# myungsub/meta-interpolation

Measured on AMD Instinct MI355X. Metric: inner-loop steps/sec, higher is better.
Workload: dtype f32 (3x3 convolutions: Winograd F(4x4) / F(2x2) on exact-f32 MFMAs, csrc/winograd4.h + winograd.hip; weight gradients and 5x5 / 7x7 / direct layers on csrc/convk*.hip: bf16x6 split operands, f32 accumulate; 51-tap op on 8-bit frames: exact integer frames x bf16x3 split taps, f32 accumulate); 1 GPU; c2_sepconv_256x448_b4_s5; plugin=sepconv, tasks_per_gpu=4, global_meta_batch=4, inner_steps=5, frame=256x448x3, inner_rule=lslr+SGD, seeded_weights=default, parallelism=task-parallel x1, 1 all-reduce of outer grads

## Files before the change

include/savfi_hip.h:

```cpp
#ifndef SAVFI_HIP_H_
#define SAVFI_HIP_H_

#include <stddef.h>
#include <stdint.h>

#ifdef __cplusplus
extern "C" {
#endif

#define SAVFI_ABI_VERSION 23

#define SAVFI_OK            0
#define SAVFI_E_NULL       (-1)
#define SAVFI_E_SHAPE      (-2)
#define SAVFI_E_UNSUPPORTED (-3)
#define SAVFI_E_TOOBIG     (-4)

int savfi_version(void);

int savfi_sepconv_fwd_f32(const float* in, const float* v, const float* h, float* out,
                          int B, int C, int Ho, int Wo, int K, void* stream);

int savfi_sepconv_bwd_f32(const float* in, const float* v, const float* h, const float* gO,
                          float* gI, float* gV, float* gH,
                          int B, int C, int Ho, int Wo, int K, void* stream);
// ... 104 lines not shown
                                    int Hs, int Ws, int oy0, int ox0, int Hw, int Ww, int align_corners, void* stream);
int savfi_upsample2x_window_bwd_masked_f32(const float* gout, const float* y, float slope, float* gin, int planes, int H, int W,
                                           int sy0, int sx0, int Hs, int Ws, int oy0, int ox0, int Hw, int Ww, int align_corners,
                                           void* stream);

int64_t savfi_conv3x3_workspace_floats(int N, int Ci, int Co, int H, int W, int pad, int mode);
int savfi_conv3x3_f32(const float* x, const float* w, const float* bias, float* out, float* workspace,
                      int N, int Ci, int Co, int H, int W, int pad, int mode, float slope, void* stream);

int64_t savfi_conv3x3_tasks_workspace_floats(int N, int T, int Ci, int Co, int H, int W, int pad, int mode);
int savfi_conv3x3_tasks_f32(const float* x, const float* w, const float* bias, float* out, float* workspace,
                            int N, int T, int Ci, int Co, int H, int W, int pad, int mode, float slope, void* stream);

int64_t savfi_conv3x3_filter_floats(int T, int Ci, int Co, int mode);
int64_t savfi_conv3x3_f4_workgroups(int N, int Ci, int Co, int H, int W, int pad, int mode);
int savfi_conv3x3_filters_form_f32(const float* w, float* u_fwd, float* u_bwd, int T, int Ci, int Co, int form, void* stream);
int savfi_conv3x3_filters_multi_form_f32(const float* const* w, float* const* u_fwd, float* const* u_bwd, const int* T, const int* Ci,
                                         const int* Co, const int* form, int n, void* stream);
int savfi_conv3x3_dgrad_masked_form_f32(const float* gy, const float* u, const float* mask, float mask_slope, float* gx, float* workspace,
                                        int N, int T, int Ci, int Co, int H, int W, int pad, int form, void* stream);
int savfi_conv3x3_filters_f32(const float* w, float* u_fwd, float* u_bwd, int T, int Ci, int Co, void* stream);
int savfi_conv3x3_filters_multi_f32(const float* const* w, float* const* u_fwd, float* const* u_bwd, const int* T, const int* Ci,
                                    const int* Co, int n, void* stream);
int64_t savfi_conv3x3_tasks_pre_workspace_floats(int N, int T, int Ci, int Co, int H, int W, int pad, int mode);
int savfi_conv3x3_tasks_pre_f32(const float* x, const float* u, const float* bias, float* out, float* workspace,
                                int N, int T, int Ci, int Co, int H, int W, int pad, int mode, float slope, void* stream);
int savfi_conv3x3_dgrad_masked_f32(const float* gy, const float* u, const float* mask, float mask_slope, float* gx,
                                   float* workspace, int N, int T, int Ci, int Co, int H, int W, int pad, void* stream);

int savfi_conv3x3_unit16_supported(int N, int T, int Ci, int Co, int H, int W, int pad);
// ... 5 lines not shown

int64_t savfi_conv3x3_wgrad_workspace_floats(int N, int Ci, int Co, int H, int W, int pad);
int savfi_conv3x3_wgrad_f32(const float* x, const float* gz, float* gw, float* workspace, int N, int Ci, int Co,
                            int H, int W, int pad, void* stream);

int64_t savfi_conv3x3_wgrad_tasks_workspace_floats(int N, int T, int Ci, int Co, int H, int W, int pad);
int savfi_conv3x3_wgrad_tasks_f32(const float* x, const float* gz, float* gw, float* workspace, int N, int T, int Ci,
                                  int Co, int H, int W, int pad, void* stream);

int64_t savfi_conv3x3_wgrad_wino_tasks_workspace_floats(int N, int T, int Ci, int Co, int H, int W, int pad);
int savfi_conv3x3_wgrad_wino_tasks_f32(const float* x, const float* gz, float* gw, float* workspace, int N, int T, int Ci,
                                       int Co, int H, int W, int pad, void* stream);
int64_t savfi_conv3x3_wgrad_wino_tasks_bias_workspace_floats(int N, int T, int Ci, int Co, int H, int W, int pad);
int savfi_conv3x3_wgrad_wino_tasks_bias_f32(const float* x, const float* gz, float* gw, float* gb, float* workspace, int N, int T, int Ci,
                                            int Co, int H, int W, int pad, void* stream);

int64_t savfi_convk_filter_floats(int T, int Ci, int Co, int K, int mode);
int savfi_convk_filters_f32(const float* w, float* p_fwd, float* p_bwd, int T, int Ci, int Co, int K, void* stream);
int savfi_convk_filters_multi_f32(const float* const* w, float* const* p_fwd, float* const* p_bwd, const int* T, const int* Ci,
                                  const int* Co, const int* K, int n, void* stream);
int savfi_convk_tasks_pre_f32(const float* x, const float* packed, const float* bias, float* out, int N, int T, int Ci,
                              int Co, int H, int W, int K, int pad, int mode, float slope, int precise, void* stream);
int savfi_convk_dgrad_masked_f32(const float* gy, const float* packed, const float* mask, float mask_slope, float* gx, int N, int T,
                                 int Ci, int Co, int H, int W, int K, int pad, int precise, void* stream);
int savfi_convk_tasks_pre_reflect_f32(const float* x, const float* packed, const float* bias, float* out, int N, int T, int Ci,
                                      int Co, int H, int W, int K, int pad, int mode, float slope, int precise, int reflect,
                                      void* stream);
int savfi_reflect_pad_bwd_f32(const float* gp, float* gx, int planes, int H, int W, int pad, void* stream);
int savfi_reflect_pad_bwd_add_f32(const float* gp, const float* add, float* gx, int planes, int H, int W, int pad, void* stream);
int savfi_reflect_pad_fwd_f32(const float* x, float* xp, int planes, int H, int W, int pad, void* stream);
// ... 37 lines not shown
```

meta-interpolation_amd/_hip.py:

```python
import ctypes
import os
import re
from ctypes import c_double, c_float, c_int, c_int64, c_void_p, POINTER

_PKG_DIR = os.path.dirname(os.path.abspath(__file__))
LIB_PATH = os.environ.get("SAVFI_HIP_LIB") or os.path.join(_PKG_DIR, "lib", "libsavfi_hip.so")
HEADER_PATH = os.path.join(os.path.dirname(_PKG_DIR), "include", "savfi_hip.h")

RULE_SGD, RULE_ADAM, RULE_ADAMAX_LSLR, RULE_ADAMAX_MSGD = 0, 1, 2, 3
LR_SCALAR, LR_ELEMENT = 0, 1
SSIM_RANGE_PER_ROW, SSIM_RANGE_BATCH, SSIM_RANGE_FIXED = 0, 1, 2
SEPCONV_PARTITION_WS, SEPCONV_PARTITION_X6, SEPCONV_PARTITION_FP32 = 0, 1, 2
ABI_VERSION = 23

_ERRORS = {-1: "SAVFI_E_NULL (a required pointer is NULL)",
           -2: "SAVFI_E_SHAPE (bad or inconsistent dimension)",
           -3: "SAVFI_E_UNSUPPORTED",
           -4: "SAVFI_E_TOOBIG (index arithmetic would overflow)"}


class SavfiHipError(RuntimeError):
    pass


_P = c_void_p
_PP = POINTER(c_void_p)
_I64P = POINTER(c_int64)
_FP = POINTER(c_float)
# ... 38 lines not shown
    "savfi_l1_mse_f32": [c_int, _P, _P, _P, _P, c_int, c_int64, _P],
    "savfi_l1_mse_bwd_f32": [c_int, _P, _P, _P, _P, c_int, c_int64, _P],
    "savfi_ssim_scratch_floats": [c_int, c_int, c_int, c_int],
    "savfi_ssim_loss_f32": [_P, _P, _P, _P, _P, c_int, c_int, c_int, c_int, c_int, _P],
    "savfi_ssim_loss_bwd_f32": [_P, _P, _P, _P, _P, c_int, c_int, c_int, c_int, _P],
    "savfi_psnr_ssim_scratch_bytes": [c_int, c_int, c_int, c_int],
    "savfi_psnr_ssim_f32": [_P, _P, _P, _P, _P, c_int, c_int, c_int, c_int, _P],
    "savfi_upsample2x_fwd_f32": [_P, _P, c_int, c_int, c_int, c_int, _P],
    "savfi_upsample2x_bwd_f32": [_P, _P, c_int, c_int, c_int, c_int, _P],
    "savfi_conv3x3_workspace_floats": [c_int] * 7,
    "savfi_conv3x3_f32": [_P, _P, _P, _P, _P, c_int, c_int, c_int, c_int, c_int, c_int, c_int, c_float, _P],
    "savfi_conv3x3_tasks_workspace_floats": [c_int] * 8,
    "savfi_conv3x3_tasks_f32": [_P, _P, _P, _P, _P, c_int, c_int, c_int, c_int, c_int, c_int, c_int, c_int, c_float, _P],
    "savfi_conv3x3_filter_floats": [c_int] * 4,
    "savfi_conv3x3_f4_workgroups": [c_int] * 7,
    "savfi_conv3x3_filters_form_f32": [_P, _P, _P, c_int, c_int, c_int, c_int, _P],
    "savfi_conv3x3_filters_multi_form_f32": [_P, _P, _P, _P, _P, _P, _P, c_int, _P],
    "savfi_conv3x3_dgrad_masked_form_f32": [_P, _P, _P, c_float, _P, _P, c_int, c_int, c_int, c_int, c_int, c_int, c_int, c_int, _P],
    "savfi_conv3x3_filters_f32": [_P, _P, _P, c_int, c_int, c_int, _P],
    "savfi_conv3x3_tasks_pre_workspace_floats": [c_int] * 8,
    "savfi_conv3x3_tasks_pre_f32": [_P, _P, _P, _P, _P, c_int, c_int, c_int, c_int, c_int, c_int, c_int, c_int, c_float, _P],
    "savfi_conv3x3_unit16_supported": [c_int] * 7,
    "savfi_conv3x3_in_unit16_supported": [c_int] * 7,
    "savfi_conv3x3_dgrad_in_unit16_f32": [_P, _P, _P, c_int, c_int, c_int, c_int, c_int, c_int, c_int, _P],
    "savfi_conv3x3_tasks_pre_unit16_f32": [_P, _P, _P, _P, c_int, c_int, c_int, c_int, c_int, c_int, c_int, c_float, _P],
    "savfi_conv3x3_wgrad_tasks_workspace_floats": [c_int] * 7,
    "savfi_conv3x3_wgrad_tasks_f32": [_P, _P, _P, _P, c_int, c_int, c_int, c_int, c_int, c_int, c_int, _P],
    "savfi_conv3x3_wgrad_wino_tasks_workspace_floats": [c_int] * 7,
    "savfi_conv3x3_wgrad_wino_tasks_f32": [_P, _P, _P, _P, c_int, c_int, c_int, c_int, c_int, c_int, c_int, _P],
    "savfi_conv3x3_wgrad_wino_tasks_bias_workspace_floats": [c_int] * 7,
    "savfi_conv3x3_wgrad_wino_tasks_bias_f32": [_P, _P, _P, _P, _P, c_int, c_int, c_int, c_int, c_int, c_int, c_int, _P],
    "savfi_conv3x3_wgrad_workspace_floats": [c_int] * 6,
    "savfi_conv3x3_wgrad_f32": [_P, _P, _P, _P, c_int, c_int, c_int, c_int, c_int, c_int, _P],
    "savfi_convk_filter_floats": [c_int] * 5,
    "savfi_convk_filters_f32": [_P, _P, _P, c_int, c_int, c_int, c_int, _P],
    "savfi_convk_filters_multi_f32": [_P, _P, _P, _P, _P, _P, _P, c_int, _P],
    "savfi_conv3x3_filters_multi_f32": [_P, _P, _P, _P, _P, _P, c_int, _P],
    "savfi_convk_tasks_pre_f32": [_P, _P, _P, _P] + [c_int] * 9 + [c_float, c_int, _P],
    "savfi_convk_tasks_pre_reflect_f32": [_P, _P, _P, _P] + [c_int] * 9 + [c_float, c_int, c_int, _P],
    "savfi_convk_wgrad_tasks_reflect_f32": [_P, _P, _P, _P] + [c_int] * 10 + [_P],
    "savfi_reflect_pad_bwd_f32": [_P, _P, c_int, c_int, c_int, c_int, _P],
    "savfi_reflect_pad_fwd_f32": [_P, _P, c_int, c_int, c_int, c_int, _P],
    "savfi_reflect_pad_bwd_add_f32": [_P, _P, _P, c_int, c_int, c_int, c_int, _P],
    "savfi_convk_wgrad_workspace_floats": [c_int] * 8,
    "savfi_convk_wgrad_sums_bias": [c_int] * 8,
    "savfi_convk_wgrad_tasks_bias_f32": [_P, _P, _P, _P, _P] + [c_int] * 9 + [_P],
# ... 166 lines not shown
```

meta-interpolation_amd/csrc/wgrad.hip:

```cpp
#include "common.h"

namespace {

typedef float f32x4 __attribute__((ext_vector_type(4)));

constexpr int GNT = 256;
constexpr int GCO = 32, GCI = 32, GSEG = 64;
constexpr int GP = 68;
constexpr int G_FLOATS = GCO * GP;
constexpr int X_FLOATS = 3 * GCI * GP;
constexpr int BUF_FLOATS = G_FLOATS + X_FLOATS;
constexpr int TILE_FLOATS = 2 * 2 * 9 * 256;
constexpr int LDS_FLOATS_G = (2 * BUF_FLOATS > TILE_FLOATS) ? 2 * BUF_FLOATS : TILE_FLOATS;

struct WgradArgs {
  const float* x;
  const float* gz;
  float* partial;
  int Ci, Co, H, W, Ho, Wo, pad, rows, nseg, nrowchunk, cibs;
  int T;
};

struct Staged {
  float g[8], x[3][8], halo;
// ... 273 lines not shown
constexpr int WW_BLOCK_FLOATS = WW_CB * WW_CB * 9;
#ifndef WW_DOUBLE
#define WW_DOUBLE 0
#endif
constexpr int WW_LDS_FLOATS = (WW_DOUBLE ? 2 : 1) * WW_BUF;

struct WWArgs {
  const float* x;
  const float* gz;
  float* partial;
  int Ci, Co, H, W, Ho, Wo, pad, T, cibs;
  int ty_cnt, tx_cnt, cpr;
  int chunks_total;
  int chunks_per_split;
  float* bias_partial;
};

}

__device__ f32x4 savfi_wg_buffer_load_x4(i32x4w rsrc, int voffset, int soffset, int aux) __asm("llvm.amdgcn.raw.buffer.load.v4f32");
__device__ f32x2w savfi_wg_buffer_load_x2(i32x4w rsrc, int voffset, int soffset, int aux) __asm("llvm.amdgcn.raw.buffer.load.v2f32");

namespace {

__device__ __forceinline__ i32x4w ww_rsrc(const float* base, unsigned bytes) {
  const unsigned long long p = reinterpret_cast<unsigned long long>(base);
  i32x4w r;
  r.x = (int)(unsigned)p; r.y = (int)(unsigned)(p >> 32); r.z = (int)bytes; r.w = 0x00020000;
  return r;
}
// ... 75 lines not shown
    t[12 + cc] = d[4 + cc] - d[12 + cc];
  }
#pragma unroll
  for (int r = 0; r < 4; ++r)
    *reinterpret_cast<f32x4*>(vbuf + (r * WW_CB + ch) * WW_PY + 4 * tl) =
        (f32x4){t[4 * r] - t[4 * r + 2], t[4 * r + 1] + t[4 * r + 2], t[4 * r + 2] - t[4 * r + 1], t[4 * r + 1] - t[4 * r + 3]};
  const float g00 = c.g[0], g01 = c.g[1], g10 = c.g[2], g11 = c.g[3];
  if (bias_acc) *bias_acc += (g00 + g01) + (g10 + g11);
  const float s0[2] = {g00, g01}, s1[2] = {g00 + g10, g01 + g11}, s2[2] = {g00 - g10, g01 - g11}, s3[2] = {g10, g11};
  *reinterpret_cast<f32x4*>(ybuf + (0 * WW_CB + ch) * WW_PY + 4 * tl) = (f32x4){s0[0], s0[0] + s0[1], s0[0] - s0[1], s0[1]};
  *reinterpret_cast<f32x4*>(ybuf + (1 * WW_CB + ch) * WW_PY + 4 * tl) = (f32x4){s1[0], s1[0] + s1[1], s1[0] - s1[1], s1[1]};
  *reinterpret_cast<f32x4*>(ybuf + (2 * WW_CB + ch) * WW_PY + 4 * tl) = (f32x4){s2[0], s2[0] + s2[1], s2[0] - s2[1], s2[1]};
  *reinterpret_cast<f32x4*>(ybuf + (3 * WW_CB + ch) * WW_PY + 4 * tl) = (f32x4){s3[0], s3[0] + s3[1], s3[0] - s3[1], s3[1]};
}

template <bool BIAS>
__global__ __launch_bounds__(256, WW_DOUBLE ? 2 : 4) void wino_wgrad3x3(WWArgs a) {
  extern __shared__ __attribute__((aligned(16))) float lds[];
  const int tid = threadIdx.x, lane = tid & 63, w = __builtin_amdgcn_readfirstlane(tid >> 6);
  const int tl = tid & 7, ch = tid >> 3;
  const int task = blockIdx.z;
  const int cob = blockIdx.y / a.cibs, cib = blockIdx.y - cob * a.cibs;
  const int q0 = blockIdx.x * a.chunks_per_split, q1 = min(q0 + a.chunks_per_split, a.chunks_total);
  const int ci = cib * WW_CB + ch, co = cob * WW_CB + ch;

  f32x4 acc[4][2][2];
#pragma unroll
  for (int c = 0; c < 4; ++c)
#pragma unroll
    for (int i = 0; i < 2; ++i)
#pragma unroll
// ... 46 lines not shown
        for (int i = 0; i < 2; ++i)
#pragma unroll
          for (int j = 0; j < 2; ++j) acc[c][i][j] = __builtin_amdgcn_mfma_f32_16x16x4f32(ya[i][c], va[j][c], acc[c][i][j], 0, 0, 0);
      __builtin_amdgcn_sched_barrier(0);
    }
  }
  __syncthreads();
  if (do_bias) {
    auto dpp = [](float v, auto ctrl) {
      return __builtin_bit_cast(float, __builtin_amdgcn_update_dpp(0, __builtin_bit_cast(int, v), decltype(ctrl)::value, 0xf, 0xf, true));
    };
    float bsum = *bias_slot();
    bsum += dpp(bsum, std::integral_constant<int, 0xB1>{});
    bsum += dpp(bsum, std::integral_constant<int, 0x4E>{});
    bsum += dpp(bsum, std::integral_constant<int, 0x141>{});
    if (tl == 0) a.bias_partial[(((size_t)task * gridDim.x + blockIdx.x) * (gridDim.y / a.cibs) + cob) * WW_CB + ch] = bsum;
  }

  const float sr = (w == 1 || w == 2) ? 0.5f : 1.f;
  float* ex = lds;
  float* out = a.partial + (((size_t)task * gridDim.x + blockIdx.x) * gridDim.y + blockIdx.y) * WW_BLOCK_FLOATS;
#pragma unroll
  for (int i = 0; i < 2; ++i) {
#pragma unroll
    for (int j = 0; j < 2; ++j) {
      f32x4 u0, u1, u2;
#pragma unroll
      for (int e = 0; e < 4; ++e) {
        const float m0 = acc[0][i][j][e], m1 = acc[1][i][j][e], m2 = acc[2][i][j][e], m3 = acc[3][i][j][e];
        const float h = 0.5f * (m1 + m2);
        u0[e] = sr * (m0 + h);
        u1[e] = sr * (0.5f * (m1 - m2));
        u2[e] = sr * (h - m3);
      }
      float* p = ex + ((w * 3) * 2 + j) * 256 + lane * 4;
      *reinterpret_cast<f32x4*>(p) = u0;
      *reinterpret_cast<f32x4*>(p + 2 * 256) = u1;
      *reinterpret_cast<f32x4*>(p + 4 * 256) = u2;
    }
    __syncthreads();
    for (int item = tid; item < 3 * 2 * 256; item += 256) {
      const int reg = item & 3, ln = (item >> 2) & 63, j = (item >> 8) & 1, b = item >> 9;
      const float* p = ex + (b * 2 + j) * 256 + ln * 4 + reg;
      const float u_0 = p[0], u_1 = p[3 * 2 * 256], u_2 = p[2 * 3 * 2 * 256], u_3 = p[3 * 3 * 2 * 256];
      const int cor = 16 * i + 4 * (ln >> 4) + reg, cic = 16 * j + (ln & 15);
      float* o = out + (cor * WW_CB + cic) * 9 + b;
      o[0] = u_0 + u_1 + u_2;
      o[3] = u_1 - u_2;
      o[6] = u_1 + u_2 - u_3;
    }
    __syncthreads();
  }
}

__global__ __launch_bounds__(256) void wino_wgrad_reduce2(const float* __restrict__ stage2, float* __restrict__ gw, int Co, int Ci,
                                                          int cibs, int ntiles, int ngroups) {
  const int e = blockIdx.x * 256 + threadIdx.x;
  if (e >= Co * Ci * 9) return;
  stage2 += (size_t)blockIdx.y * ngroups * ntiles * WW_BLOCK_FLOATS;
  gw += (size_t)blockIdx.y * Co * Ci * 9;
  const int k = e % 9, ci = (e / 9) % Ci, co = e / (9 * Ci);
// ... 56 lines not shown
  if (!ww_plan(p, N, T, Ci, Co, H, W, pad)) return SAVFI_E_SHAPE;
  return p.partial_floats + p.stage2_floats;
}

extern "C" int64_t savfi_conv3x3_wgrad_wino_tasks_bias_workspace_floats(int N, int T, int Ci, int Co, int H, int W, int pad) {
  const int64_t base = savfi_conv3x3_wgrad_wino_tasks_workspace_floats(N, T, Ci, Co, H, W, pad);
  if (base < 0) return base;
  WWPlan p;
  ww_plan(p, N, T, Ci, Co, H, W, pad);
  return base + (int64_t)T * p.nsplit * p.cobs * WW_CB;
}

static int wino_wgrad_tasks(const float* x, const float* gz, float* gw, float* gb, float* workspace, int N, int T, int Ci, int Co, int H,
                            int W, int pad, void* stream);

extern "C" int savfi_conv3x3_wgrad_wino_tasks_f32(const float* x, const float* gz, float* gw, float* workspace, int N, int T,
                                                  int Ci, int Co, int H, int W, int pad, void* stream) {
  return wino_wgrad_tasks(x, gz, gw, nullptr, workspace, N, T, Ci, Co, H, W, pad, stream);
}

extern "C" int savfi_conv3x3_wgrad_wino_tasks_bias_f32(const float* x, const float* gz, float* gw, float* gb, float* workspace, int N, int T,
                                                       int Ci, int Co, int H, int W, int pad, void* stream) {
  if (!gb) return SAVFI_E_NULL;
  return wino_wgrad_tasks(x, gz, gw, gb, workspace, N, T, Ci, Co, H, W, pad, stream);
}

static int wino_wgrad_tasks(const float* x, const float* gz, float* gw, float* gb, float* workspace, int N, int T, int Ci, int Co, int H,
                            int W, int pad, void* stream) {
  if (!x || !gz || !gw || !workspace) return SAVFI_E_NULL;
  if (N <= 0 || T <= 0 || N % T != 0 || Ci <= 0 || Co <= 0 || H <= 0 || W <= 0) return SAVFI_E_SHAPE;
  if (pad != 0 && pad != 1) return SAVFI_E_UNSUPPORTED;
  WWPlan p;
  if (!ww_plan(p, N, T, Ci, Co, H, W, pad)) return SAVFI_E_SHAPE;
  if ((int64_t)Ci * H * W >= ((int64_t)1 << 28) || (int64_t)Co * p.Ho * p.Wo >= ((int64_t)1 << 28)) return SAVFI_E_TOOBIG;
  if (p.ngroups > 65535 || (int64_t)p.cobs * p.cibs > 65535 || (int64_t)Co * Ci * 9 > 0x7fffffffLL || T > 65535) return SAVFI_E_TOOBIG;
  hipStream_t st = (hipStream_t)stream;
  constexpr size_t lds = (size_t)WW_LDS_FLOATS * sizeof(float), lds_bias = lds + 256 * sizeof(float);
  static uint32_t attr_done = 0, attr_done_b = 0;
  if (int e = gb ? savfi_ensure_dynamic_lds((const void*)wino_wgrad3x3<true>, lds_bias, attr_done_b)
                 : savfi_ensure_dynamic_lds((const void*)wino_wgrad3x3<false>, lds, attr_done)) return e;
  float* bias_partial = gb ? workspace + p.partial_floats + p.stage2_floats : nullptr;
  WWArgs a{x, gz, workspace, Ci, Co, H, W, p.Ho, p.Wo, pad, T, p.cibs, p.ty_cnt, p.tx_cnt, p.cpr, p.chunks_total, p.chunks_per_split,
           bias_partial};
  if (gb) hipLaunchKernelGGL(wino_wgrad3x3<true>, dim3(p.nsplit, p.cobs * p.cibs, T), dim3(256), lds_bias, st, a);
  else hipLaunchKernelGGL(wino_wgrad3x3<false>, dim3(p.nsplit, p.cobs * p.cibs, T), dim3(256), lds, st, a);
  if (int e = savfi_launch_status()) return e;
  if (gb) {
    hipLaunchKernelGGL(wino_wgrad_bias_reduce, dim3(savfi_cdiv(Co, 64), T), dim3(64), 0, st, bias_partial, gb, Co, p.cobs, p.nsplit);
    if (int e = savfi_launch_status()) return e;
  }
  const int ntiles = p.cobs * p.cibs;
  const size_t block_floats = (size_t)ntiles * WW_BLOCK_FLOATS;
  float* stage2 = workspace + p.partial_floats;
  if (p.ngroups == 1) {
    hipLaunchKernelGGL(wino_wgrad_reduce2, dim3(savfi_cdiv(Co * Ci * 9, 256), T), dim3(256), 0, st, workspace, gw, Co, Ci, p.cibs, ntiles,
                       p.nsplit);
    return savfi_launch_status();
  }
  hipLaunchKernelGGL(wgrad_reduce1, dim3((unsigned)((block_floats / 4 + 255) / 256), p.ngroups, T), dim3(256), 0, st, workspace,
                     stage2, block_floats, p.nsplit);
  if (int e = savfi_launch_status()) return e;
// ... 5 lines not shown
```

meta-interpolation_amd/csrc/winograd.hip:

```cpp
#include "common.h"
#include <type_traits>

typedef float f32x4 __attribute__((ext_vector_type(4)));
typedef int i32x4 __attribute__((ext_vector_type(4)));
__device__ f32x4 savfi_raw_buffer_load_x4(i32x4 rsrc, int voffset, int soffset, int aux) __asm("llvm.amdgcn.raw.buffer.load.v4f32");
typedef float f32x2 __attribute__((ext_vector_type(2)));
__device__ void savfi_raw_buffer_store_x2(f32x2 data, i32x4 rsrc, int voffset, int soffset, int aux) __asm("llvm.amdgcn.raw.buffer.store.v2f32");
__device__ f32x2 savfi_raw_buffer_load_x2(i32x4 rsrc, int voffset, int soffset, int aux) __asm("llvm.amdgcn.raw.buffer.load.v2f32");
__device__ float savfi_raw_buffer_load_x1(i32x4 rsrc, int voffset, int soffset, int aux) __asm("llvm.amdgcn.raw.buffer.load.f32");
__device__ void savfi_raw_buffer_store_x1(float data, i32x4 rsrc, int voffset, int soffset, int aux) __asm("llvm.amdgcn.raw.buffer.store.f32");
__device__ void savfi_raw_buffer_store_x4(f32x4 data, i32x4 rsrc, int voffset, int soffset, int aux) __asm("llvm.amdgcn.raw.buffer.store.v4f32");

namespace {

#include "winograd4.h"

constexpr int WNT = 256;
constexpr int TILES_WG = 64;
constexpr int COB = 32;
constexpr int CIB = 4;
#ifndef WINO_VS
#define WINO_VS 80
#endif
constexpr int VS = WINO_VS;
// ... 478 lines not shown
  acc = acc > 0.f ? acc : slope * acc;
  if (mask) acc = mask[e] > 0.f ? acc : acc * mask_slope;
  out[e] = acc;
}

int round_up(int v, int m) { return (v + m - 1) / m * m; }

#ifndef SAVFI_WINO_SPLIT_SLOTS
#define SAVFI_WINO_SPLIT_SLOTS 512
#endif

struct WinoPlan {
  int K, I, KP, IP, off, Ho, Wo, th, tw, tile_shift, nsplit, chunks_per_split;
  int64_t u_floats, partial_floats;
  bool f4;
};

inline bool f4_for(int K, int I, int form) { return form != 2 && w4::use_f4(K, I); }
inline int kp_for(int K, int I, int form) { return f4_for(K, I, form) ? w4::kp_of(K) : (K + 2 * CIB - 1) / (2 * CIB) * (2 * CIB); }
inline int ip_for(int K, int I, int form) { return f4_for(K, I, form) ? w4::ip_of(I) : (I + COB - 1) / COB * COB; }
inline int64_t u_floats_for(int K, int I, int form) { return (int64_t)(f4_for(K, I, form) ? w4::PTS : 16) * kp_for(K, I, form) * ip_for(K, I, form); }

bool make_plan(WinoPlan& p, int N, int Ci, int Co, int H, int W, int pad, int mode) {
  const int form = (mode & 2) ? 2 : 0;
  mode &= 1;
  p.K = mode == 0 ? Ci : Co;
  p.I = mode == 0 ? Co : Ci;
  p.f4 = f4_for(p.K, p.I, form);
  p.KP = kp_for(p.K, p.I, form);
  p.IP = ip_for(p.K, p.I, form);
  p.off = mode == 0 ? pad : 2 - pad;
  p.Ho = H + 2 * p.off - 2;
  p.Wo = W + 2 * p.off - 2;
  if (p.Ho <= 0 || p.Wo <= 0) return false;
  if (p.f4) {
    const int ty4 = savfi_cdiv(p.Ho, 4), tx4 = savfi_cdiv(p.Wo, 4);
    int64_t best4 = -1;
#ifndef SAVFI_W4_TS_ORDER
#define SAVFI_W4_TS_ORDER 2
#endif
#if SAVFI_W4_TS_ORDER == 0
    for (int s : {3, 4, 2, 5, 1, 0}) {
#elif SAVFI_W4_TS_ORDER == 1
    for (int s : {4, 3, 5, 2, 1, 0}) {
#else
    for (int s : {5, 4, 3, 2, 1, 0}) {
#endif
      const int64_t blocks = (int64_t)savfi_cdiv(ty4, w4::TT >> s) * savfi_cdiv(tx4, 1 << s);
      if (best4 < 0 || blocks < best4) { best4 = blocks; p.tile_shift = s; }
    }
    p.th = savfi_cdiv(ty4, w4::TT >> p.tile_shift);
    p.tw = savfi_cdiv(tx4, 1 << p.tile_shift);
    const int nchunk4 = p.KP / w4::KC;
    const int64_t wgs4 = (int64_t)p.th * p.tw * (p.IP / w4::COB) * N;
    int want4 = (int)(SAVFI_WINO_SPLIT_SLOTS / (wgs4 > 0 ? wgs4 : 1));
    want4 = (want4 < 2 || nchunk4 < 32) ? 1 : (want4 > 8 ? 8 : want4);
    int cps4 = savfi_cdiv(nchunk4, want4);
    if (cps4 < 8) cps4 = nchunk4 < 8 ? nchunk4 : 8;
    p.chunks_per_split = cps4;
    p.nsplit = savfi_cdiv(nchunk4, cps4);
    p.u_floats = u_floats_for(p.K, p.I, form);
    p.partial_floats = p.nsplit > 1 ? (int64_t)p.nsplit * N * p.I * p.Ho * p.Wo : 0;
    return true;
  }
  const int ty = savfi_cdiv(p.Ho, 2), tx = savfi_cdiv(p.Wo, 2);
  int64_t best = -1;
  for (int s : {4, 3, 5, 2}) {
// ... 41 lines not shown
  if (N <= 0 || T <= 0 || N % T != 0 || Ci <= 0 || Co <= 0 || H <= 0 || W <= 0) return SAVFI_E_SHAPE;
  if ((mode & ~3) || (pad != 0 && pad != 1)) return SAVFI_E_UNSUPPORTED;
  WinoPlan p;
  if (!make_plan(p, N, Ci, Co, H, W, pad, mode)) return SAVFI_E_SHAPE;
  return (int64_t)T * p.u_floats + p.partial_floats;
}

extern "C" int64_t savfi_conv3x3_f4_workgroups(int N, int Ci, int Co, int H, int W, int pad, int mode) {
  if (N <= 0 || Ci <= 0 || Co <= 0 || H <= 0 || W <= 0) return SAVFI_E_SHAPE;
  if ((mode & ~3) || (pad != 0 && pad != 1)) return SAVFI_E_UNSUPPORTED;
  WinoPlan p;
  if (!make_plan(p, N, Ci, Co, H, W, pad, mode)) return SAVFI_E_SHAPE;
  return p.f4 ? (int64_t)p.th * p.tw * (p.IP / w4::COB) * p.nsplit * N : 0;
}

extern "C" int64_t savfi_conv3x3_workspace_floats(int N, int Ci, int Co, int H, int W, int pad, int mode) {
  return savfi_conv3x3_tasks_workspace_floats(N, 1, Ci, Co, H, W, pad, mode);
}

namespace {

template <int VECW, int IN16, bool MASK>
int launch_wino4(const w4::W4Args& a4, int64_t wgs4, hipStream_t st) {
  static uint32_t configured = 0;
  constexpr size_t lds4 = (size_t)w4::LDS_FLOATS * sizeof(float);
  auto kern = w4::wino4_conv3x3<VECW, IN16, MASK>;
  if (int rc = savfi_ensure_dynamic_lds(reinterpret_cast<const void*>(kern), lds4, configured)) return rc;
  hipLaunchKernelGGL(kern, dim3((unsigned)wgs4), dim3(256), lds4, st, a4);
  return savfi_launch_status();
}

int launch_conv(const WinoPlan& p, const float* x, const float* U, const float* bias, float* out, float* partial, int N, int T,
                int H, int W, int mode, float slope, hipStream_t st, const float* mask = nullptr, float mask_slope = 1.f,
                int out_unit16 = 0, int in_unit16 = 0) {
  if (p.f4) {
    const int64_t wgs4 = (int64_t)p.th * p.tw * (p.IP / w4::COB) * p.nsplit * N;
    if (wgs4 > 0x7fffffffLL || T > 65535) return SAVFI_E_TOOBIG;
    if (mask && (out_unit16 || in_unit16)) return SAVFI_E_UNSUPPORTED;
    if (p.nsplit > 1 && (out_unit16 || in_unit16 || !partial)) return SAVFI_E_UNSUPPORTED;
    if (in_unit16 && ((p.off != 1 && p.off != 2) || p.Wo % 2 != 0)) return SAVFI_E_UNSUPPORTED;
    w4::W4Args a4{x, U, (mode & 1) == 0 ? bias : nullptr, out, p.K, p.I, p.KP, p.IP, H, W, p.Ho, p.Wo, p.off, p.th, p.tw, slope,
                  p.tile_shift, T, N, p.nsplit > 1 ? nullptr : mask, mask_slope, out_unit16, p.nsplit, p.chunks_per_split, partial};
    const int vecw = p.Wo % 4 == 0 ? 4 : (p.Wo % 2 == 0 ? 2 : 1);
    auto go = [&](auto kern) { return kern(a4, wgs4, st); };
    if (in_unit16 && p.off == 1) return vecw == 4 ? go(launch_wino4<4, 2, false>) : go(launch_wino4<2, 2, false>);
    if (in_unit16) return vecw == 4 ? go(launch_wino4<4, 3, false>) : go(launch_wino4<2, 3, false>);
    if (p.nsplit > 1) {
      const int rc = vecw == 4 ? go(launch_wino4<4, 0, false>) : vecw == 2 ? go(launch_wino4<2, 0, false>) : go(launch_wino4<1, 0, false>);
      if (rc != SAVFI_OK) return rc;
      const size_t total = (size_t)N * p.I * p.Ho * p.Wo;
      hipLaunchKernelGGL(wino_split_reduce, dim3((unsigned)((total + 255) / 256)), dim3(256), 0, st, partial, (mode & 1) == 0 ? bias : nullptr, out,
                         p.nsplit, total, p.I, p.Ho * p.Wo, slope, T, mask, mask_slope);
      return savfi_launch_status();
    }
    if (mask) return vecw == 4 ? go(launch_wino4<4, 0, true>) : vecw == 2 ? go(launch_wino4<2, 0, true>) : go(launch_wino4<1, 0, true>);
    return vecw == 4 ? go(launch_wino4<4, 0, false>) : vecw == 2 ? go(launch_wino4<2, 0, false>) : go(launch_wino4<1, 0, false>);
  }
// ... 189 lines not shown
```

meta-interpolation_amd/csrc/winograd4.h:

```cpp
#pragma once

namespace w4 {

constexpr int TT = 32;
constexpr int COB = 32;
constexpr int KC = 8;
constexpr int PTS = 36;
constexpr int VBUF = PTS * KC * TT;
constexpr int XBUF = PTS * 16 * TT;
constexpr int LDS_FLOATS = XBUF > 2 * VBUF ? XBUF : 2 * VBUF;
#ifndef SAVFI_W4_MAXC
#define SAVFI_W4_MAXC 512
#endif

__host__ __device__ inline bool use_f4(int K, int I) { return K <= SAVFI_W4_MAXC && I <= SAVFI_W4_MAXC; }
__host__ __device__ inline int kp_of(int K) { return (K + KC - 1) / KC * KC; }
__host__ __device__ inline int ip_of(int I) { return (I + COB - 1) / COB * COB; }

__device__ __forceinline__ void g_rows(const float (&g)[3], float (&t)[6]) {
  const float s = g[0] + g[2];
  const float s4 = fmaf(4.f, g[2], g[0]);
  t[0] = 0.25f * g[0];
  t[1] = (s + g[1]) * (-1.f / 6.f);
  t[2] = (s - g[1]) * (-1.f / 6.f);
// ... 44 lines not shown
      else blk[16 * 64 + lane * 2 + (v - 16)] = o[c];
    }
  }
  __syncthreads();
  const int chunk = bx >> 1, s2 = bx & 1, ncob = IP / COB, cob0 = 2 * (by % nI);
  if (4 * bx >= KP) return;
#pragma unroll
  for (int it = 0; it < 8 * 18 * 64 / 4 / 256; ++it) {
    const int e = (it * 256 + threadIdx.x) * 4;
    const int blkid = e / (18 * 64), off = e - blkid * (18 * 64);
    const int cobq = cob0 + (blkid >> 2), wv = blkid & 3;
    if (cobq >= ncob) continue;
    float* dst = U + ((((size_t)chunk * ncob + cobq) * 4 + wv) * 2 + s2) * (18 * 64) + off;
    *reinterpret_cast<f32x4*>(dst) = *reinterpret_cast<const f32x4*>(stage + e);
  }
}

struct W4Args {
  const float* x;
  const float* U;
  const float* bias;
  float* out;
  int K, I, KP, IP, H, W, Ho, Wo, off, tiles_y, tiles_x;
  float slope;
  int tile_shift;
  int T, N;
  const float* mask;
  float mask_slope;
  int out_unit16;
  int nsplit, chunks_per_split;
  float* partial;
};

__device__ __forceinline__ i32x4 w4_rsrc(const void* base, unsigned bytes) {
  const unsigned long long p = reinterpret_cast<unsigned long long>(base);
  i32x4 r;
  r.x = (int)(unsigned)p;
  r.y = (int)(unsigned)(p >> 32);
  r.z = (int)bytes;
  r.w = 0x00020000;
  return r;
}

__device__ __forceinline__ i32x4 w4_uniform(i32x4 r) {
  r.x = __builtin_amdgcn_readfirstlane(r.x); r.y = __builtin_amdgcn_readfirstlane(r.y);
  r.z = __builtin_amdgcn_readfirstlane(r.z); r.w = __builtin_amdgcn_readfirstlane(r.w);
// ... 47 lines not shown

  const int nblk = a.IP / COB;
  int tb, cob, n, sp;
  {
    const unsigned flat = blockIdx.x, nwg = gridDim.x;
    const unsigned ntb = (unsigned)(a.tiles_y * a.tiles_x);
    const unsigned xcd = flat & 7u, q8 = nwg >> 3, rem = nwg & 7u;
    unsigned item = xcd * q8 + min(xcd, rem) + (flat >> 3);
    cob = (int)(item % (unsigned)nblk);
    item /= (unsigned)nblk;
    tb = (int)(item % ntb);
    item /= ntb;
    sp = (int)(item % (unsigned)a.nsplit);
    n = (int)(item / (unsigned)a.nsplit);
  }
  const int tby = tb / a.tiles_x, tbx = tb - tby * a.tiles_x;
  const int i0 = cob * COB;
  const int task = a.T > 1 ? n % a.T : 0;
  const size_t cplane = (size_t)a.H * a.W;
  const float* xp = a.x + (size_t)n * a.K * cplane;
  const int tsh = a.tile_shift, tbw = 1 << tsh, tbh = TT >> tsh;

  const int tl = lane & 31, kc = 2 * w + (lane >> 5);
  const int y0 = 4 * (tby * tbh + (tl >> tsh)) - a.off, x0 = 4 * (tbx * tbw + (tl & (tbw - 1))) - a.off;
  constexpr int WC = IN16 ? IN16 - 1 : 0;
  unsigned pv[6], pn[IN16 ? 6 : 1], pn2[IN16 == 2 ? 6 : 1];
  unsigned long long shl = 0, colm[6] = {~0ull, ~0ull, ~0ull, ~0ull, ~0ull, ~0ull};
  int partial = 0;
  unsigned chunk_bytes;
  unsigned plane_b;
  if constexpr (IN16) {
    plane_b = 64u;
    chunk_bytes = KC * 64u;
    auto at = [&](bool row, int y, int x) {
      return (row && x >= 0 && x < a.W) ? (unsigned)((y * (a.W >> 4) + (x >> 4)) * a.K) * 64u + (unsigned)(x & 15) * 4u + (unsigned)kc * 64u : 0x80000000u;
    };
#pragma unroll
    for (int r = 0; r < 6; ++r) {
      const int y = y0 + r;
// ... 186 lines not shown
  __builtin_amdgcn_s_waitcnt(0);
  __syncthreads();

  const int split = a.nsplit > 1 ? 1 : 0;
  float* const obase = split ? a.partial + (size_t)sp * a.N * a.I * a.Ho * a.Wo : a.out;
  float bvals[2][2];
#pragma unroll
  for (int cb = 0; cb < 2; ++cb)
#pragma unroll
    for (int qq = 0; qq < 2; ++qq) {
      const int i = i0 + 16 * cb + (tid >> 5) + 8 * qq;
      bvals[cb][qq] = (a.bias && split == 0 && i < a.I) ? a.bias[task * a.I + i] : 0.f;
    }

  const int otl = tid & 31, och = tid >> 5;
  const int oy = 4 * (tby * tbh + (otl >> tsh)), ox = 4 * (tbx * tbw + (otl & (tbw - 1)));
  const unsigned oplane = (unsigned)(a.Ho * a.Wo) * 4u;
  constexpr int NS = 4 / VECW;
  unsigned ooff[4][NS];
#pragma unroll
  for (int r = 0; r < 4; ++r)
#pragma unroll
    for (int e = 0; e < NS; ++e) {
      const int x = ox + e * VECW;
      const bool ok = oy + r < a.Ho && x < a.Wo;
      if (a.out_unit16) ooff[r][e] = ok ? (unsigned)(((oy + r) * (a.Wo >> 4) + (x >> 4)) * a.I) * 64u + (unsigned)(x & 15) * 4u : 0x80000000u;
      else ooff[r][e] = ok ? (unsigned)((oy + r) * a.Wo + x) * 4u + (unsigned)(lane >> 5) * oplane : 0x80000000u;
    }
  auto pair_rsrc = [&](const float* base, int cb, int qq) {
    const int ie = i0 + 16 * cb + 2 * w + 8 * qq;
    const int have = a.I - ie < 0 ? 0 : (a.I - ie > 2 ? 2 : a.I - ie);
// ... 96 lines not shown
```

meta-interpolation_amd/hip_ops.py:

```python
import collections
import functools
import ctypes
import os
import threading

import torch
from torch.autograd.function import once_differentiable

from . import _hip

_PASS = threading.local()


def set_double_backward(value):
    _PASS.double_backward = bool(value)


def double_backward():
    return getattr(_PASS, 'double_backward', False)


class _VoxelWarp(torch.autograd.Function):
    @staticmethod
    def forward(ctx, frames, x3):
# ... 743 lines not shown

WINO4_MIN_WORKGROUPS = 180
WINO4_MIN_PIXELS = 400


@functools.lru_cache(maxsize=None)
def _conv3x3_name(Ci, Co, what):
    f4 = int(_hip.lib().savfi_conv3x3_f4_workgroups(1, int(Ci), int(Co), 8, 8, 1, 0)) > 0
    return ("conv3x3f4_" if f4 else "conv3x3_") + what


@functools.lru_cache(maxsize=4096)
def wino4_workgroups(N, Ci, Co, H, W, pad, mode=0):
    n = int(_hip.lib().savfi_conv3x3_f4_workgroups(int(N), int(Ci), int(Co), int(H), int(W), int(pad), int(mode)))
    return max(n, 0)


def _layer(x_shape, w_shape, stride, padding, dilation, groups=1):
    geo = _conv_geometry(w_shape, stride, padding, dilation, groups)
    if geo is None or len(x_shape) != 4:
        return None
    return (int(x_shape[0]), int(w_shape[-3]), int(w_shape[-4]), int(x_shape[2]), int(x_shape[3])) + geo


def _form2(N, Ci, Co, H, W, pad):
    n = wino4_workgroups(int(N), int(Ci), int(Co), int(H), int(W), int(pad))
    if n <= 0:
        return False
    return n < WINO4_MIN_WORKGROUPS or (H + 2 * pad - 2) * (W + 2 * pad - 2) < WINO4_MIN_PIXELS

# ... 1097 lines not shown
```

Measured before the change: 246.9 inner-loop steps/sec.

## Add flat Winograd tile mapping and direct single-split wgrad output

Adds a flat tile-to-workgroup mapping for the F(4x4) Winograd forward kernel. Tiles are packed linearly in blocks of TT whenever that needs fewer workgroups than the shaped 2D tiling, which cuts padding waste on frames whose tile grid does not divide evenly. It also lets the Winograd weight-gradient kernel write gw and gb straight to the output when there is only one split, skipping the partial buffer and the reduce launches. Both are on by default with runtime toggles, and they add per-thread div/mod index math plus bounds checks in the kernels.

```diff
diff --git a/include/savfi_hip.h b/include/savfi_hip.h
--- a/include/savfi_hip.h
+++ b/include/savfi_hip.h
@@ -8,7 +8,7 @@
 extern "C" {
 #endif
 
-#define SAVFI_ABI_VERSION 23
+#define SAVFI_ABI_VERSION 24
 
 #define SAVFI_OK            0
 #define SAVFI_E_NULL       (-1)
@@ -143,6 +143,10 @@
 
 int64_t savfi_conv3x3_filter_floats(int T, int Ci, int Co, int mode);
 int64_t savfi_conv3x3_f4_workgroups(int N, int Ci, int Co, int H, int W, int pad, int mode);
+int64_t savfi_conv3x3_f4_launch_workgroups(int N, int Ci, int Co, int H, int W, int pad, int mode);
+int savfi_conv3x3_f4_set_flat_tiles(int on);
+int savfi_conv3x3_f4_tile_plan(int ty4, int tx4, int* flat, int* tile_shift, int* shaped_blocks);
+int savfi_conv3x3_f4_tile_map(int ty4, int tx4, int* ty, int* tx, int cap);
 int savfi_conv3x3_filters_form_f32(const float* w, float* u_fwd, float* u_bwd, int T, int Ci, int Co, int form, void* stream);
 int savfi_conv3x3_filters_multi_form_f32(const float* const* w, float* const* u_fwd, float* const* u_bwd, const int* T, const int* Ci,
                                          const int* Co, const int* form, int n, void* stream);
@@ -178,6 +182,8 @@
 int64_t savfi_conv3x3_wgrad_wino_tasks_bias_workspace_floats(int N, int T, int Ci, int Co, int H, int W, int pad);
 int savfi_conv3x3_wgrad_wino_tasks_bias_f32(const float* x, const float* gz, float* gw, float* gb, float* workspace, int N, int T, int Ci,
                                             int Co, int H, int W, int pad, void* stream);
+int savfi_conv3x3_wgrad_wino_splits(int N, int T, int Ci, int Co, int H, int W, int pad);
+int savfi_conv3x3_wgrad_wino_set_direct(int on);
 
 int64_t savfi_convk_filter_floats(int T, int Ci, int Co, int K, int mode);
 int savfi_convk_filters_f32(const float* w, float* p_fwd, float* p_bwd, int T, int Ci, int Co, int K, void* stream);
diff --git a/meta-interpolation_amd/_hip.py b/meta-interpolation_amd/_hip.py
--- a/meta-interpolation_amd/_hip.py
+++ b/meta-interpolation_amd/_hip.py
@@ -11,7 +11,7 @@
 LR_SCALAR, LR_ELEMENT = 0, 1
 SSIM_RANGE_PER_ROW, SSIM_RANGE_BATCH, SSIM_RANGE_FIXED = 0, 1, 2
 SEPCONV_PARTITION_WS, SEPCONV_PARTITION_X6, SEPCONV_PARTITION_FP32 = 0, 1, 2
-ABI_VERSION = 23
+ABI_VERSION = 24
 
 _ERRORS = {-1: "SAVFI_E_NULL (a required pointer is NULL)",
            -2: "SAVFI_E_SHAPE (bad or inconsistent dimension)",
@@ -80,6 +80,10 @@
     "savfi_conv3x3_tasks_f32": [_P, _P, _P, _P, _P, c_int, c_int, c_int, c_int, c_int, c_int, c_int, c_int, c_float, _P],
     "savfi_conv3x3_filter_floats": [c_int] * 4,
     "savfi_conv3x3_f4_workgroups": [c_int] * 7,
+    "savfi_conv3x3_f4_launch_workgroups": [c_int] * 7,
+    "savfi_conv3x3_f4_set_flat_tiles": [c_int],
+    "savfi_conv3x3_f4_tile_plan": [c_int, c_int, POINTER(c_int), POINTER(c_int), POINTER(c_int)],
+    "savfi_conv3x3_f4_tile_map": [c_int, c_int, POINTER(c_int), POINTER(c_int), c_int],
     "savfi_conv3x3_filters_form_f32": [_P, _P, _P, c_int, c_int, c_int, c_int, _P],
     "savfi_conv3x3_filters_multi_form_f32": [_P, _P, _P, _P, _P, _P, _P, c_int, _P],
     "savfi_conv3x3_dgrad_masked_form_f32": [_P, _P, _P, c_float, _P, _P, c_int, c_int, c_int, c_int, c_int, c_int, c_int, c_int, _P],
@@ -96,6 +100,8 @@
     "savfi_conv3x3_wgrad_wino_tasks_f32": [_P, _P, _P, _P, c_int, c_int, c_int, c_int, c_int, c_int, c_int, _P],
     "savfi_conv3x3_wgrad_wino_tasks_bias_workspace_floats": [c_int] * 7,
     "savfi_conv3x3_wgrad_wino_tasks_bias_f32": [_P, _P, _P, _P, _P, c_int, c_int, c_int, c_int, c_int, c_int, c_int, _P],
+    "savfi_conv3x3_wgrad_wino_splits": [c_int] * 7,
+    "savfi_conv3x3_wgrad_wino_set_direct": [c_int],
     "savfi_conv3x3_wgrad_workspace_floats": [c_int] * 6,
     "savfi_conv3x3_wgrad_f32": [_P, _P, _P, _P, c_int, c_int, c_int, c_int, c_int, c_int, _P],
     "savfi_convk_filter_floats": [c_int] * 5,
diff --git a/meta-interpolation_amd/csrc/wgrad.hip b/meta-interpolation_amd/csrc/wgrad.hip
--- a/meta-interpolation_amd/csrc/wgrad.hip
+++ b/meta-interpolation_amd/csrc/wgrad.hip
@@ -1,4 +1,5 @@
 #include "common.h"
+#include <atomic>
 
 namespace {
 
@@ -311,6 +312,8 @@
   int chunks_total;
   int chunks_per_split;
   float* bias_partial;
+  float* gw;
+  float* gb;
 };
 
 }
@@ -416,7 +419,7 @@
   *reinterpret_cast<f32x4*>(ybuf + (3 * WW_CB + ch) * WW_PY + 4 * tl) = (f32x4){s3[0], s3[0] + s3[1], s3[0] - s3[1], s3[1]};
 }
 
-template <bool BIAS>
+template <bool BIAS, bool DIRECT>
 __global__ __launch_bounds__(256, WW_DOUBLE ? 2 : 4) void wino_wgrad3x3(WWArgs a) {
   extern __shared__ __attribute__((aligned(16))) float lds[];
   const int tid = threadIdx.x, lane = tid & 63, w = __builtin_amdgcn_readfirstlane(tid >> 6);
@@ -493,12 +496,19 @@
     bsum += dpp(bsum, std::integral_constant<int, 0xB1>{});
     bsum += dpp(bsum, std::integral_constant<int, 0x4E>{});
     bsum += dpp(bsum, std::integral_constant<int, 0x141>{});
-    if (tl == 0) a.bias_partial[(((size_t)task * gridDim.x + blockIdx.x) * (gridDim.y / a.cibs) + cob) * WW_CB + ch] = bsum;
+    if (tl == 0) {
+      if constexpr (DIRECT) { if (co < a.Co) a.gb[(size_t)task * a.Co + co] = bsum; }
+      else a.bias_partial[(((size_t)task * gridDim.x + blockIdx.x) * (gridDim.y / a.cibs) + cob) * WW_CB + ch] = bsum;
+    }
   }
 
   const float sr = (w == 1 || w == 2) ? 0.5f : 1.f;
   float* ex = lds;
-  float* out = a.partial + (((size_t)task * gridDim.x + blockIdx.x) * gridDim.y + blockIdx.y) * WW_BLOCK_FLOATS;
+  constexpr bool direct = DIRECT;
+  float* out = direct ? a.gw + (((size_t)task * a.Co + cob * WW_CB) * a.Ci + cib * WW_CB) * 9
+                      : a.partial + (((size_t)task * gridDim.x + blockIdx.x) * gridDim.y + blockIdx.y) * WW_BLOCK_FLOATS;
+  const int orow = direct ? a.Ci * 9 : WW_CB * 9;
+  const int colim = direct ? a.Co - cob * WW_CB : WW_CB, cilim = direct ? a.Ci - cib * WW_CB : WW_CB;
 #pragma unroll
   for (int i = 0; i < 2; ++i) {
 #pragma unroll
@@ -523,7 +533,8 @@
       const float* p = ex + (b * 2 + j) * 256 + ln * 4 + reg;
       const float u_0 = p[0], u_1 = p[3 * 2 * 256], u_2 = p[2 * 3 * 2 * 256], u_3 = p[3 * 3 * 2 * 256];
       const int cor = 16 * i + 4 * (ln >> 4) + reg, cic = 16 * j + (ln & 15);
-      float* o = out + (cor * WW_CB + cic) * 9 + b;
+      if (DIRECT && (cor >= colim || cic >= cilim)) continue;
+      float* o = out + cor * orow + cic * 9 + b;
       o[0] = u_0 + u_1 + u_2;
       o[3] = u_1 - u_2;
       o[6] = u_1 + u_2 - u_3;
@@ -610,6 +621,17 @@
 static int wino_wgrad_tasks(const float* x, const float* gz, float* gw, float* gb, float* workspace, int N, int T, int Ci, int Co, int H,
                             int W, int pad, void* stream);
 
+static std::atomic<int> g_ww_direct{1};
+extern "C" int savfi_conv3x3_wgrad_wino_set_direct(int on) { return g_ww_direct.exchange(on ? 1 : 0); }
+
+extern "C" int savfi_conv3x3_wgrad_wino_splits(int N, int T, int Ci, int Co, int H, int W, int pad) {
+  if (N <= 0 || T <= 0 || N % T != 0 || Ci <= 0 || Co <= 0 || H <= 0 || W <= 0) return SAVFI_E_SHAPE;
+  if (pad != 0 && pad != 1) return SAVFI_E_UNSUPPORTED;
+  WWPlan p;
+  if (!ww_plan(p, N, T, Ci, Co, H, W, pad)) return SAVFI_E_SHAPE;
+  return p.nsplit;
+}
+
 extern "C" int savfi_conv3x3_wgrad_wino_tasks_f32(const float* x, const float* gz, float* gw, float* workspace, int N, int T,
                                                   int Ci, int Co, int H, int W, int pad, void* stream) {
   return wino_wgrad_tasks(x, gz, gw, nullptr, workspace, N, T, Ci, Co, H, W, pad, stream);
@@ -632,15 +654,20 @@
   if (p.ngroups > 65535 || (int64_t)p.cobs * p.cibs > 65535 || (int64_t)Co * Ci * 9 > 0x7fffffffLL || T > 65535) return SAVFI_E_TOOBIG;
   hipStream_t st = (hipStream_t)stream;
   constexpr size_t lds = (size_t)WW_LDS_FLOATS * sizeof(float), lds_bias = lds + 256 * sizeof(float);
-  static uint32_t attr_done = 0, attr_done_b = 0;
-  if (int e = gb ? savfi_ensure_dynamic_lds((const void*)wino_wgrad3x3<true>, lds_bias, attr_done_b)
-                 : savfi_ensure_dynamic_lds((const void*)wino_wgrad3x3<false>, lds, attr_done)) return e;
   float* bias_partial = gb ? workspace + p.partial_floats + p.stage2_floats : nullptr;
+  const bool direct = p.nsplit == 1 && g_ww_direct.load(std::memory_order_relaxed) != 0;
   WWArgs a{x, gz, workspace, Ci, Co, H, W, p.Ho, p.Wo, pad, T, p.cibs, p.ty_cnt, p.tx_cnt, p.cpr, p.chunks_total, p.chunks_per_split,
-           bias_partial};
-  if (gb) hipLaunchKernelGGL(wino_wgrad3x3<true>, dim3(p.nsplit, p.cobs * p.cibs, T), dim3(256), lds_bias, st, a);
-  else hipLaunchKernelGGL(wino_wgrad3x3<false>, dim3(p.nsplit, p.cobs * p.cibs, T), dim3(256), lds, st, a);
-  if (int e = savfi_launch_status()) return e;
+           bias_partial, direct ? gw : nullptr, direct ? gb : nullptr};
+  static uint32_t attr_done[4] = {0, 0, 0, 0};
+  auto go = [&](auto kern, size_t bytes, uint32_t& done) {
+    if (int e = savfi_ensure_dynamic_lds((const void*)kern, bytes, done)) return e;
+    hipLaunchKernelGGL(kern, dim3(p.nsplit, p.cobs * p.cibs, T), dim3(256), bytes, st, a);
+    return savfi_launch_status();
+  };
+  const int rc = gb ? (direct ? go(wino_wgrad3x3<true, true>, lds_bias, attr_done[3]) : go(wino_wgrad3x3<true, false>, lds_bias, attr_done[2]))
+                    : (direct ? go(wino_wgrad3x3<false, true>, lds, attr_done[1]) : go(wino_wgrad3x3<false, false>, lds, attr_done[0]));
+  if (rc != SAVFI_OK) return rc;
+  if (direct) return SAVFI_OK;
   if (gb) {
     hipLaunchKernelGGL(wino_wgrad_bias_reduce, dim3(savfi_cdiv(Co, 64), T), dim3(64), 0, st, bias_partial, gb, Co, p.cobs, p.nsplit);
     if (int e = savfi_launch_status()) return e;
diff --git a/meta-interpolation_amd/csrc/winograd.hip b/meta-interpolation_amd/csrc/winograd.hip
--- a/meta-interpolation_amd/csrc/winograd.hip
+++ b/meta-interpolation_amd/csrc/winograd.hip
@@ -1,4 +1,5 @@
 #include "common.h"
+#include <atomic>
 #include <type_traits>
 
 typedef float f32x4 __attribute__((ext_vector_type(4)));
@@ -516,7 +517,34 @@
   int K, I, KP, IP, off, Ho, Wo, th, tw, tile_shift, nsplit, chunks_per_split;
   int64_t u_floats, partial_floats;
   bool f4;
+  int ty4, tx4;
+  bool flat;
+  int flat_blocks;
 };
+
+std::atomic<int> g_w4_flat_tiles{1};
+
+inline void w4_tile_plan(int ty4, int tx4, int& tile_shift, int& th, int& tw, bool& flat, int& flat_blocks) {
+  int64_t best4 = -1;
+#ifndef SAVFI_W4_TS_ORDER
+#define SAVFI_W4_TS_ORDER 2
+#endif
+#if SAVFI_W4_TS_ORDER == 0
+  for (int s : {3, 4, 2, 5, 1, 0}) {
+#elif SAVFI_W4_TS_ORDER == 1
+  for (int s : {4, 3, 5, 2, 1, 0}) {
+#else
+  for (int s : {5, 4, 3, 2, 1, 0}) {
+#endif
+    const int64_t blocks = (int64_t)savfi_cdiv(ty4, w4::TT >> s) * savfi_cdiv(tx4, 1 << s);
+    if (best4 < 0 || blocks < best4) { best4 = blocks; tile_shift = s; }
+  }
+  th = savfi_cdiv(ty4, w4::TT >> tile_shift);
+  tw = savfi_cdiv(tx4, 1 << tile_shift);
+  const int64_t fb = ((int64_t)ty4 * tx4 + w4::TT - 1) / w4::TT;
+  flat = g_w4_flat_tiles.load(std::memory_order_relaxed) != 0 && fb < (int64_t)th * tw && (int64_t)ty4 * tx4 <= 0x3fffffffLL;
+  flat_blocks = (int)fb;
+}
 
 inline bool f4_for(int K, int I, int form) { return form != 2 && w4::use_f4(K, I); }
 inline int kp_for(int K, int I, int form) { return f4_for(K, I, form) ? w4::kp_of(K) : (K + 2 * CIB - 1) / (2 * CIB) * (2 * CIB); }
@@ -536,23 +564,9 @@
   p.Wo = W + 2 * p.off - 2;
   if (p.Ho <= 0 || p.Wo <= 0) return false;
   if (p.f4) {
-    const int ty4 = savfi_cdiv(p.Ho, 4), tx4 = savfi_cdiv(p.Wo, 4);
-    int64_t best4 = -1;
-#ifndef SAVFI_W4_TS_ORDER
-#define SAVFI_W4_TS_ORDER 2
-#endif
-#if SAVFI_W4_TS_ORDER == 0
-    for (int s : {3, 4, 2, 5, 1, 0}) {
-#elif SAVFI_W4_TS_ORDER == 1
-    for (int s : {4, 3, 5, 2, 1, 0}) {
-#else
-    for (int s : {5, 4, 3, 2, 1, 0}) {
-#endif
-      const int64_t blocks = (int64_t)savfi_cdiv(ty4, w4::TT >> s) * savfi_cdiv(tx4, 1 << s);
-      if (best4 < 0 || blocks < best4) { best4 = blocks; p.tile_shift = s; }
-    }
-    p.th = savfi_cdiv(ty4, w4::TT >> p.tile_shift);
-    p.tw = savfi_cdiv(tx4, 1 << p.tile_shift);
+    p.ty4 = savfi_cdiv(p.Ho, 4);
+    p.tx4 = savfi_cdiv(p.Wo, 4);
+    w4_tile_plan(p.ty4, p.tx4, p.tile_shift, p.th, p.tw, p.flat, p.flat_blocks);
     const int nchunk4 = p.KP / w4::KC;
     const int64_t wgs4 = (int64_t)p.th * p.tw * (p.IP / w4::COB) * N;
     int want4 = (int)(SAVFI_WINO_SPLIT_SLOTS / (wgs4 > 0 ? wgs4 : 1));
@@ -624,6 +638,46 @@
   return p.f4 ? (int64_t)p.th * p.tw * (p.IP / w4::COB) * p.nsplit * N : 0;
 }
 
+static inline int64_t w4_launch_blocks(const WinoPlan& p) { return p.flat ? (int64_t)p.flat_blocks : (int64_t)p.th * p.tw; }
+
+extern "C" int64_t savfi_conv3x3_f4_launch_workgroups(int N, int Ci, int Co, int H, int W, int pad, int mode) {
+  if (N <= 0 || Ci <= 0 || Co <= 0 || H <= 0 || W <= 0) return SAVFI_E_SHAPE;
+  if ((mode & ~3) || (pad != 0 && pad != 1)) return SAVFI_E_UNSUPPORTED;
+  WinoPlan p;
+  if (!make_plan(p, N, Ci, Co, H, W, pad, mode)) return SAVFI_E_SHAPE;
+  return p.f4 ? w4_launch_blocks(p) * (p.IP / w4::COB) * p.nsplit * N : 0;
+}
+
+extern "C" int savfi_conv3x3_f4_set_flat_tiles(int on) { return g_w4_flat_tiles.exchange(on ? 1 : 0); }
+
+extern "C" int savfi_conv3x3_f4_tile_plan(int ty4, int tx4, int* flat, int* tile_shift, int* shaped_blocks) {
+  if (ty4 <= 0 || tx4 <= 0 || (int64_t)ty4 * tx4 > 0x3fffffffLL) return SAVFI_E_SHAPE;
+  int s, th, tw, fb;
+  bool fl;
+  w4_tile_plan(ty4, tx4, s, th, tw, fl, fb);
+  if (flat) *flat = fl ? 1 : 0;
+  if (tile_shift) *tile_shift = s;
+  if (shaped_blocks) *shaped_blocks = th * tw;
+  return fl ? fb : th * tw;
+}
+
+extern "C" int savfi_conv3x3_f4_tile_map(int ty4, int tx4, int* ty, int* tx, int cap) {
+  if (!ty || !tx) return SAVFI_E_NULL;
+  int fl, s;
+  const int blocks = savfi_conv3x3_f4_tile_plan(ty4, tx4, &fl, &s, nullptr);
+  if (blocks < 0) return blocks;
+  if ((int64_t)blocks * w4::TT > cap) return SAVFI_E_TOOBIG;
+  const int tw = savfi_cdiv(tx4, 1 << s);
+  for (int b = 0; b < blocks; ++b)
+    for (int slot = 0; slot < w4::TT; ++slot) {
+      int y, x;
+      const bool have = w4::tile_of(b, slot, s, tw, ty4, tx4, fl, y, x);
+      ty[b * w4::TT + slot] = have ? y : -1;
+      tx[b * w4::TT + slot] = have ? x : -1;
+    }
+  return blocks * w4::TT;
+}
+
 extern "C" int64_t savfi_conv3x3_workspace_floats(int N, int Ci, int Co, int H, int W, int pad, int mode) {
   return savfi_conv3x3_tasks_workspace_floats(N, 1, Ci, Co, H, W, pad, mode);
 }
@@ -644,13 +698,14 @@
                 int H, int W, int mode, float slope, hipStream_t st, const float* mask = nullptr, float mask_slope = 1.f,
                 int out_unit16 = 0, int in_unit16 = 0) {
   if (p.f4) {
-    const int64_t wgs4 = (int64_t)p.th * p.tw * (p.IP / w4::COB) * p.nsplit * N;
+    const int64_t wgs4 = w4_launch_blocks(p) * (p.IP / w4::COB) * p.nsplit * N;
     if (wgs4 > 0x7fffffffLL || T > 65535) return SAVFI_E_TOOBIG;
     if (mask && (out_unit16 || in_unit16)) return SAVFI_E_UNSUPPORTED;
     if (p.nsplit > 1 && (out_unit16 || in_unit16 || !partial)) return SAVFI_E_UNSUPPORTED;
     if (in_unit16 && ((p.off != 1 && p.off != 2) || p.Wo % 2 != 0)) return SAVFI_E_UNSUPPORTED;
-    w4::W4Args a4{x, U, (mode & 1) == 0 ? bias : nullptr, out, p.K, p.I, p.KP, p.IP, H, W, p.Ho, p.Wo, p.off, p.th, p.tw, slope,
-                  p.tile_shift, T, N, p.nsplit > 1 ? nullptr : mask, mask_slope, out_unit16, p.nsplit, p.chunks_per_split, partial};
+    w4::W4Args a4{x, U, (mode & 1) == 0 ? bias : nullptr, out, p.K, p.I, p.KP, p.IP, H, W, p.Ho, p.Wo, p.off, p.flat ? p.flat_blocks : p.th,
+                  p.flat ? 1 : p.tw, slope, p.tile_shift, T, N, p.nsplit > 1 ? nullptr : mask, mask_slope, out_unit16, p.nsplit,
+                  p.chunks_per_split, partial, p.ty4, p.tx4, p.flat ? 1 : 0};
     const int vecw = p.Wo % 4 == 0 ? 4 : (p.Wo % 2 == 0 ? 2 : 1);
     auto go = [&](auto kern) { return kern(a4, wgs4, st); };
     if (in_unit16 && p.off == 1) return vecw == 4 ? go(launch_wino4<4, 2, false>) : go(launch_wino4<2, 2, false>);
diff --git a/meta-interpolation_amd/csrc/winograd4.h b/meta-interpolation_amd/csrc/winograd4.h
--- a/meta-interpolation_amd/csrc/winograd4.h
+++ b/meta-interpolation_amd/csrc/winograd4.h
@@ -82,6 +82,19 @@
     float* dst = U + ((((size_t)chunk * ncob + cobq) * 4 + wv) * 2 + s2) * (18 * 64) + off;
     *reinterpret_cast<f32x4*>(dst) = *reinterpret_cast<const f32x4*>(stage + e);
   }
+}
+
+__host__ __device__ inline bool tile_of(int tb, int slot, int tile_shift, int blocks_x, int ty4, int tx4, int flat, int& ty, int& tx) {
+  if (flat) {
+    const int f = TT * tb + slot;
+    ty = f / tx4;
+    tx = f - ty * tx4;
+    return f < ty4 * tx4;
+  }
+  const int tby = tb / blocks_x, tbx = tb - tby * blocks_x;
+  ty = tby * (TT >> tile_shift) + (slot >> tile_shift);
+  tx = (tbx << tile_shift) + (slot & ((1 << tile_shift) - 1));
+  return ty < ty4 && tx < tx4;
 }
 
 struct W4Args {
@@ -98,6 +111,7 @@
   int out_unit16;
   int nsplit, chunks_per_split;
   float* partial;
+  int ty4, tx4, flat;
 };
 
 __device__ __forceinline__ i32x4 w4_rsrc(const void* base, unsigned bytes) {
@@ -175,15 +189,19 @@
     sp = (int)(item % (unsigned)a.nsplit);
     n = (int)(item / (unsigned)a.nsplit);
   }
-  const int tby = tb / a.tiles_x, tbx = tb - tby * a.tiles_x;
   const int i0 = cob * COB;
   const int task = a.T > 1 ? n % a.T : 0;
   const size_t cplane = (size_t)a.H * a.W;
   const float* xp = a.x + (size_t)n * a.K * cplane;
-  const int tsh = a.tile_shift, tbw = 1 << tsh, tbh = TT >> tsh;
 
   const int tl = lane & 31, kc = 2 * w + (lane >> 5);
-  const int y0 = 4 * (tby * tbh + (tl >> tsh)) - a.off, x0 = 4 * (tbx * tbw + (tl & (tbw - 1))) - a.off;
+  int y0, x0;
+  {
+    int ty, tx;
+    const bool have = tile_of(tb, tl, a.tile_shift, a.tiles_x, a.ty4, a.tx4, a.flat, ty, tx);
+    y0 = 4 * ty - a.off; x0 = 4 * tx - a.off;
+    if (a.flat && !have) { y0 = a.H; x0 = 0; }
+  }
   constexpr int WC = IN16 ? IN16 - 1 : 0;
   unsigned pv[6], pn[IN16 ? 6 : 1], pn2[IN16 == 2 ? 6 : 1];
   unsigned long long shl = 0, colm[6] = {~0ull, ~0ull, ~0ull, ~0ull, ~0ull, ~0ull};
@@ -400,7 +418,13 @@
     }
 
   const int otl = tid & 31, och = tid >> 5;
-  const int oy = 4 * (tby * tbh + (otl >> tsh)), ox = 4 * (tbx * tbw + (otl & (tbw - 1)));
+  int oy, ox;
+  {
+    int ty, tx;
+    const bool have = tile_of(tb, otl, a.tile_shift, a.tiles_x, a.ty4, a.tx4, a.flat, ty, tx);
+    oy = 4 * ty; ox = 4 * tx;
+    if (a.flat && !have) oy = a.Ho;
+  }
   const unsigned oplane = (unsigned)(a.Ho * a.Wo) * 4u;
   constexpr int NS = 4 / VECW;
   unsigned ooff[4][NS];
diff --git a/meta-interpolation_amd/hip_ops.py b/meta-interpolation_amd/hip_ops.py
--- a/meta-interpolation_amd/hip_ops.py
+++ b/meta-interpolation_amd/hip_ops.py
@@ -781,6 +781,19 @@
 def wino4_workgroups(N, Ci, Co, H, W, pad, mode=0):
     n = int(_hip.lib().savfi_conv3x3_f4_workgroups(int(N), int(Ci), int(Co), int(H), int(W), int(pad), int(mode)))
     return max(n, 0)
+
+
+def wino4_launch_workgroups(N, Ci, Co, H, W, pad, mode=0):
+    n = int(_hip.lib().savfi_conv3x3_f4_launch_workgroups(int(N), int(Ci), int(Co), int(H), int(W), int(pad), int(mode)))
+    return max(n, 0)
+
+
+def set_wino4_flat_tiles(on):
+    return bool(_hip.lib().savfi_conv3x3_f4_set_flat_tiles(1 if on else 0))
+
+
+def set_wgrad_wino_direct(on):
+    return bool(_hip.lib().savfi_conv3x3_wgrad_wino_set_direct(1 if on else 0))
 
 
 def _layer(x_shape, w_shape, stride, padding, dilation, groups=1):
```

New measurement: 246.1 inner-loop steps/sec. Within noise of the previous version (-0.3%).
